# TencentYoutuResearch/NeRF-Loc

Measured on AMD Instinct MI355X. Metric: rendered rays/sec (4096 rays×128 samples, 256-wide MLP) at 1/2/4/8 MI355X, higher is better.
Workload: dtype f16mx (neural-point kernel, conv_out and feat_mlp.0: fp16 hi.hi + two MX-FP6 cross terms, 1.5 MFMA-equivalents per product; every other GEMM 3-term split-bf16 or split-fp16; fp32 accumulate; meets 1e-4)

## Files before the change

### nerf_loc_amd/csrc/tgemm.hip

```cpp
#include "common.h"
#include "mfma.h"

namespace {

__device__ __forceinline__ void tg_split8_f16(const float (&v)[8], nl_bf16x8& hi, nl_bf16x8& lo) {
  nl_f16x8 h, l;
#pragma unroll
  for (int t = 0; t < 8; ++t) { const _Float16 x = (_Float16)v[t]; h[t] = x; l[t] = (_Float16)(v[t] - (float)x); }
  hi = __builtin_bit_cast(nl_bf16x8, h);
  lo = __builtin_bit_cast(nl_bf16x8, l);
}

__device__ __forceinline__ int tg_find_seg(const NlGemmArgs& a, int k0) {
  int s = 0;
#pragma unroll
  for (int j = 1; j < NL_GEMM_MAX_SEG; ++j) s += (k0 >= a.kstart[j]) ? 1 : 0;
  return __builtin_amdgcn_readfirstlane(s);
}

#ifdef TG_TRACE
__device__ unsigned long long tg_trace[64];
#define TG_T(i)                                                                                      \
  do {                                                                                               \
    if (NRT == 8 && EPI == NL_EPI_LNSLAB && blockIdx.x == 0 && wave == 0 && a.Kpad > 512) {          \
// ... 839 lines not shown
    nl_f32x2 s = {0.f, 0.f};
#pragma unroll
    for (int r = 0; r < 16; r += 2) s = __builtin_elementwise_fma(nl_lrelu2(nl_f32x2{acc[rt][r], acc[rt][r + 1]} + bb), wp[r >> 1], s);
    float p = s[0] + s[1];
    p += __shfl_xor(p, 32, 64);
    if (hh == 0) red[wave * 256 + 32 * rt + j] = p;
  }
  __syncthreads();
  const int wpr = S >> 5, rays_wg = NW / wpr, R = M / S;
  for (int i = tid; i < rays_wg * 256; i += 64 * NW) {
    const int q = i >> 8, c = i & 255;
    float sum = 0.f;
    for (int w = 0; w < wpr; ++w) sum += red[(q * wpr + w) * 256 + c];
    const int ray = grp * rays_wg + q;
    if (w2) reinterpret_cast<float*>(hcsT)[c * HB + nbuf + q] = sum;
    else if (ray < R) hc[(size_t)ray * 256 + c] = sum;
  }
  __syncthreads();
  P = Pn;
  if (w2) {
    if (nbuf == 0) grp0 = grp;
    nbuf += rays_wg;
    const bool last = grp + (int)gridDim.x >= ngroups;
    if (nbuf + rays_wg > HB || last) {
      const int n = tid % npad, set = tid / npad;
      if (set < 2 && n < C) {
        float a[8];
#pragma unroll
        for (int i = 0; i < 8; ++i) a[i] = 0.f;
#pragma unroll 8
        for (int k = 0; k < 256; ++k) {
          const float b = w2[(size_t)k * npad + n];
          const float4 h0 = hcsT[k * (HB / 4) + set * 2], h1 = hcsT[k * (HB / 4) + set * 2 + 1];
          a[0] = fmaf(h0.x, b, a[0]); a[1] = fmaf(h0.y, b, a[1]); a[2] = fmaf(h0.z, b, a[2]); a[3] = fmaf(h0.w, b, a[3]);
          a[4] = fmaf(h1.x, b, a[4]); a[5] = fmaf(h1.y, b, a[5]); a[6] = fmaf(h1.z, b, a[6]); a[7] = fmaf(h1.w, b, a[7]);
        }
        const float b2 = w2[(size_t)256 * npad + n];
#pragma unroll
        for (int i = 0; i < 8; ++i) {
          const int slot = set * 8 + i;
          const int ray = (grp0 + (slot / rays_wg) * (int)gridDim.x) * rays_wg + slot % rays_wg;
          if (slot < nbuf && ray < R) feat[(size_t)ray * C + n] = fmaf(wsum[ray], b2, a[i]);
        }
      }
      nbuf = 0;
      __syncthreads();
    }
  }
  }
}


constexpr int TGC1_NRT = 2, TGC1_NW = 4, TGC1_D = 3, TGC1_NB = TGC1_D + 1, TGC1_NCH = 24;
template <bool X3, bool F16 = false>
__global__ __launch_bounds__(64 * TGC1_NW, 4) void tgemm_conv1_kernel(const NlGemmArgs a, const char* __restrict__ p_bst, float* __restrict__ p_c, const float* __restrict__ p_zeros,
                                                                      const float* __restrict__ p_bias) {
  constexpr int NRT = TGC1_NRT, NW = TGC1_NW, D = TGC1_D, NB = TGC1_NB, NCH = TGC1_NCH;
  constexpr int PARTS = X3 ? 2 : 1;
  constexpr int CHB = 4 * NRT * 1024;
  constexpr int SLOTB = PARTS * 2 * NRT * 1024;
  constexpr int PPW = SLOTB / 1024 / NW;
  static_assert(PPW * NW * 1024 == SLOTB, "pieces per wave");
  __shared__ uint4 lds_all[NB * SLOTB / 16 + NRT * 8 * 2 + 8];
  float* sbias = reinterpret_cast<float*>(lds_all + NB * SLOTB / 16);

  const int tid = threadIdx.x, lane = tid & 63, wave = __builtin_amdgcn_readfirstlane(tid >> 6);
  const int hh = lane >> 5, j = lane & 31;
  const int tile = blockIdx.x * NW + wave;
  const int m = tile * 32 + j;
  const bool mok = m < a.M;
  const int q = m / a.So, t = m - q * a.So;

  for (int i = tid; i < NRT * 32; i += 64 * NW) sbias[i] = (p_bias && i < a.N) ? p_bias[i] : 0.f;

  const __amdgpu_buffer_rsrc_t rw = __builtin_amdgcn_make_buffer_rsrc((void*)p_bst, 0, 0x7fffffff, 0x00020000);
  const unsigned lane16 = lane * 16;
  auto stage_piece = [&](auto Cc, auto Ic) __attribute__((always_inline)) {
    constexpr int c = decltype(Cc)::value, slot = c % NB, i = decltype(Ic)::value;
    const int pp = wave + NW * i;
    unsigned so = (unsigned)c * CHB + pp * 1024;
    asm volatile("" : "+s"(so));
    __builtin_amdgcn_raw_ptr_buffer_load_lds(rw, (__attribute__((address_space(3))) void*)(lds_all + (slot * SLOTB) / 16 + pp * 64), 16, lane16, so, 0, 0);
  };
  auto stage = [&](auto Cc) __attribute__((always_inline)) {
    nl_static_for<PPW>([&](auto Ic) __attribute__((always_inline)) { stage_piece(Cc, Ic); });
  };
  const NlGemmSeg& g0 = a.seg[0];
  const int frg = __builtin_amdgcn_readfirstlane(g0.frag);
  const int fr0 = frg == 3 ? 1 : frg;
  const int cstride0 = fr0 == 1 ? 1024 : 32;
  const float* P0[3]; int okm[3];
#pragma unroll
  for (int tp = 0; tp < 3; ++tp) {
    const int i = t + tp - 1;
    const bool ok = mok && i >= 0 && i < a.Li;
    const int row = q * a.Li + i;
    okm[tp] = ok ? 1 : 0;
    const float* f = fr0 == 1 ? g0.ptr + ((size_t)(row >> 5) * (g0.k >> 4)) * 512 + ((row & 31) + 32 * hh) * 4 : g0.ptr + (size_t)row * g0.ld + (fr0 == 2 ? 4 : 8) * hh;
    P0[tp] = ok ? f : p_zeros;
  }
  auto act_off = [](int fr, int pc) __attribute__((always_inline)) { return fr == 1 ? 256 * pc : 16 * (pc >> 1) + (fr == 2 ? 8 : 4) * (pc & 1); };
  float4 raw[D][4];
  auto load_act = [&](auto Cc) __attribute__((always_inline)) {
    constexpr int c = decltype(Cc)::value, tp = c % 3, cb = c / 3;
    const float* p = P0[tp] + okm[tp] * (cb * cstride0);
#pragma unroll
    for (int pc = 0; pc < 4; ++pc) raw[c % D][pc] = *(const float4*)(p + act_off(fr0, pc));
  };
  auto load_act_piece = [&](auto Cc, auto Pc) __attribute__((always_inline)) {
    constexpr int c = decltype(Cc)::value, tp = c % 3, cb = c / 3, pc = decltype(Pc)::value;
    const float* p = P0[tp] + okm[tp] * (cb * cstride0);
    raw[c % D][pc] = *(const float4*)(p + act_off(fr0, pc));
  };

  nl_f32x16 acc[NRT];
#pragma unroll
  for (int rt = 0; rt < NRT; ++rt)
#pragma unroll
    for (int r = 0; r < 16; ++r) acc[rt][r] = 0.f;

  nl_static_for<D>([&](auto Cc) __attribute__((always_inline)) { stage(Cc); load_act(Cc); });

#if defined(TG_TRACE) && defined(TG_TRACE_C1)
#define TGC1_T(k) do { if (blockIdx.x == 0 && wave == 0 && g >= 8 && g < 14) { const unsigned long long t_ = __builtin_readcyclecounter(); if (lane == 0) tg_trace[5 * (g - 8) + (k)] = t_; } } while (0)
#else
#define TGC1_T(k)
#endif
  nl_static_for<NCH>([&](auto Gc) __attribute__((always_inline)) {
    constexpr int g = decltype(Gc)::value;
    TGC1_T(0);
    constexpr int nlater = (g + D - 1 < NCH ? D - 1 : NCH - 1 - g);
    constexpr int later = nlater * (PPW + 4);
    nl_wait_vmcnt<later>();
    TGC1_T(1);
    __syncthreads();
    TGC1_T(2);
    nl_bf16x8 bh[2], bl[2];
    {
      const float4 (&rw4)[4] = raw[g % D];
      if (fr0 == 1) {
        bh[0] = __builtin_bit_cast(nl_bf16x8, rw4[0]); bl[0] = __builtin_bit_cast(nl_bf16x8, rw4[1]);
        bh[1] = __builtin_bit_cast(nl_bf16x8, rw4[2]); bl[1] = __builtin_bit_cast(nl_bf16x8, rw4[3]);
      } else {
#pragma unroll
        for (int ks = 0; ks < 2; ++ks) {
          const float v[8] = {rw4[2 * ks].x, rw4[2 * ks].y, rw4[2 * ks].z, rw4[2 * ks].w, rw4[2 * ks + 1].x, rw4[2 * ks + 1].y, rw4[2 * ks + 1].z, rw4[2 * ks + 1].w};
          if constexpr (F16) tg_split8_f16(v, bh[ks], bl[ks]); else nl_split8<X3>(v, bh[ks], bl[ks]);
        }
      }
    }
    auto mem_slot = [&](auto Mc) __attribute__((always_inline)) {
      constexpr int m = decltype(Mc)::value;
      if constexpr (g + D < NCH) {
        if constexpr (m < PPW) stage_piece(std::integral_constant<int, g + D>{}, Mc);
        else if constexpr (m < PPW + 4) load_act_piece(std::integral_constant<int, g + D>{}, std::integral_constant<int, m - PPW>{});
      }
    };
    TGC1_T(3);
    const nl_bf16x8* L = reinterpret_cast<const nl_bf16x8*>(lds_all + ((g % NB) * SLOTB) / 16);
    nl_static_for<2 * NRT>([&](auto Tc) __attribute__((always_inline)) {
        constexpr int tt = decltype(Tc)::value, ks = tt / NRT, rt = tt % NRT;
        const nl_bf16x8 ah = L[((0 * 2 + ks) * NRT + rt) * 64 + lane];
        if (X3) {
          const nl_bf16x8 al = L[((1 * 2 + ks) * NRT + rt) * 64 + lane];
          acc[rt] = nl_mfma<F16>(al, bh[ks], acc[rt]);
          acc[rt] = nl_mfma<F16>(ah, bl[ks], acc[rt]);
        }
        acc[rt] = nl_mfma<F16>(ah, bh[ks], acc[rt]);
        mem_slot(std::integral_constant<int, (tt < 2 ? 2 * tt : 2 + tt)>{});
        if constexpr (tt < 2) mem_slot(std::integral_constant<int, 2 * tt + 1>{});
        __builtin_amdgcn_sched_barrier(0);
      });
    __builtin_amdgcn_sched_barrier(0);
    TGC1_T(4);
  });

  __syncthreads();
  float* red = sbias + NRT * 32;
  float s1 = 0.f;
#pragma unroll
  for (int rt = 0; rt < NRT; ++rt)
#pragma unroll
    for (int gq = 0; gq < 4; ++gq) {
      const int n = 32 * rt + 8 * gq + 4 * hh;
      const float4 b4 = *(const float4*)(sbias + n);
      nl_f32x2 p0, p1;
      nl_bias_sum4(acc[rt][4 * gq + 0], acc[rt][4 * gq + 1], acc[rt][4 * gq + 2], acc[rt][4 * gq + 3], b4, p0, p1, s1);
      acc[rt][4 * gq + 0] = p0[0]; acc[rt][4 * gq + 1] = p0[1]; acc[rt][4 * gq + 2] = p1[0]; acc[rt][4 * gq + 3] = p1[1];
    }
  s1 = wave_sum(s1);
  if (lane == 0) red[wave] = s1;
  __syncthreads();
  float tot = 0.f;
#pragma unroll
  for (int w = 0; w < NW; ++w) tot += red[w];
  const float cnt = (float)a.So * (float)a.N;
  const float mean = tot / cnt;
  float s2;
  {
    nl_f32x2 sp = {0.f, 0.f};
#pragma unroll
    for (int rt = 0; rt < NRT; ++rt)
#pragma unroll
      for (int r = 0; r < 16; r += 2) nl_sumsq_dev2(sp, acc[rt][r], acc[rt][r + 1], mean);
    s2 = sp[0] + sp[1];
  }
  s2 = wave_sum(s2);
  if (lane == 0) red[NW + wave] = s2;
// ... 359 lines not shown
        if constexpr (FEAT) {
#pragma unroll
          for (int rt = 0; rt < 8; ++rt) {
#pragma unroll
            for (int gq = 0; gq < 4; ++gq) {
              const int n = 32 * rt + 8 * gq + 4 * hh;
              const float4 b4 = *(const float4*)(stab + 512 + n);
              float (&v)[16] = fa[rt % (QUERY ? 4 : 8)];
              const nl_f32x2 l0 = nl_lrelu2(nl_f32x2{acc[rt][4 * gq], acc[rt][4 * gq + 1]} + nl_f32x2{b4.x, b4.y});
              const nl_f32x2 l1 = nl_lrelu2(nl_f32x2{acc[rt][4 * gq + 2], acc[rt][4 * gq + 3]} + nl_f32x2{b4.z, b4.w});
              v[4 * gq] = l0[0]; v[4 * gq + 1] = l0[1]; v[4 * gq + 2] = l1[0]; v[4 * gq + 3] = l1[1];
            }
#pragma unroll
            for (int r = 0; r < 16; ++r) acc[rt][r] = 0.f;
            if (rt >= 2) store_fa(rt - 2, rFT, row1k);
            __builtin_amdgcn_sched_barrier(0);
          }
        }
      }
      if constexpr (kd == CK_BL && Geo::last(c)) {
        const unsigned brow = mok_c ? (unsigned)m_c * 128u + 16u * hh : DROP;
#pragma unroll
        for (int gq = 0; gq < 4; ++gq)
          __builtin_amdgcn_raw_buffer_store_b128(__builtin_bit_cast(nl_u32x4, nl_f32x4{acc[0][4 * gq], acc[0][4 * gq + 1], acc[0][4 * gq + 2], acc[0][4 * gq + 3]}), rBL,
                                                 brow + 32 * gq, 0, 0);
        zero_acc(I0{}, I2{});
      }
      if constexpr (kd == CK_Q && Geo::last(c)) {
#pragma unroll
        for (int rt = 0; rt < 4; ++rt)
#pragma unroll
          for (int r = 0; r < 16; ++r) { fa[rt % (QUERY ? 4 : 8)][r] = qacc[rt % (QUERY ? 4 : 1)][r]; qacc[rt % (QUERY ? 4 : 1)][r] = 0.f; }
      }
      CHAIN_T(2);
    });
#ifdef CHAIN_TRACE
    ++trace_it;
#endif
    prev_row = QUERY ? (mok_c ? (unsigned)m_c * 512u + 16u * hh : DROP) : row1k;
    m_c = m_n; mm_c = mm_n; mok_c = mok_n;
    tile = tile_next;
    if (tile >= ntiles) break;
  }
  if constexpr (QUERY) {
#pragma unroll
    for (int q = 0; q < 16; ++q) store_fa(q, rFA, prev_row);
  } else if constexpr (FEAT) {
#pragma unroll
    for (int q = 8; q < 32; ++q) store_fa(q, rFT, prev_row);
  }
  nl_wait_vmcnt<0>();
}

}

int nl_tgemm_nrt(int N) { return N <= 64 ? 2 : (N <= 128 ? 4 : 8); }
size_t nl_tgemm_mx_image_bytes(int Kpad) { return (size_t)((Kpad / 32 + 1) / 2) * TGMX_IMG; }
size_t nl_tgemm_stream_bytes(int Kpad, int N) { return (size_t)(Kpad / 32) * 4 * nl_tgemm_nrt(N) * 1024; }

bool nl_tgemm_supported(const NlGemmArgs& a, int precision) {
  if (precision == NL_PREC_F16X3_INTERNAL && (a.epi != NL_EPI_NONE || a.tile_map)) return false;
  if (a.act == NL_ACT_LRELU_MASK && (a.epi != NL_EPI_NONE || a.So > 0 || (!a.ep_maskin && (!a.ep_res || (a.ep_ldres & 3) || (((size_t)a.ep_res) & 15))))) return false;
  if ((a.ep_maskout || a.ep_maskin) && (a.epi != NL_EPI_NONE || a.So > 0 || a.tile_map)) return false;
  if (a.ep_tab && (a.epi != NL_EPI_NONE || a.So > 0 || a.tile_map || a.act == NL_ACT_LRELU_MASK || !a.ep_tabidx || a.ep_tabK <= 0 || (a.ep_ldtab & 3) ||
                   (((size_t)a.ep_tab) & 15)))
    return false;
  if (a.tile_map && (a.epi != NL_EPI_NONE || a.So > 0 || !a.tile_count)) return false;
  if (precision == NL_PREC_F32 || !a.Bst || a.N > 256 || (a.N & 3) || (a.ldc & 3) || (((size_t)a.C) & 15) || a.M <= 0 || !a.zeros) return false;
  if (a.epi == NL_EPI_LNROW && (a.N != 32 * nl_tgemm_nrt(a.N) || a.So > 0 || !a.ep_res || (a.ep_ldres & 3) || (((size_t)a.ep_res) & 15))) return false;
  if (a.epi == NL_EPI_LNSLAB && ((a.So != 192 && a.So != 96 && a.So != 128 && a.So != 64 && a.So != 32 && a.So != 16) || a.M % a.So || a.Li != a.So || a.ostride != 1 || a.ooff != 0 || !a.ep_gamma || !a.ep_beta)) return false;
  for (int s = 0; s < a.nseg; ++s) {
    const NlGemmSeg& g = a.seg[s];
    if (!g.vec || (g.k & 31) || g.rdiv > 1 || g.ld < g.k || g.ntap < 1) return false;
    if (g.frag && precision == NL_PREC_F16X3_INTERNAL) return false;
  }
  return true;
}

static bool nl_tgemm_mx_supported(const NlGemmArgs& a, int precision) {
  if (precision != NL_PREC_BF16X3 || !a.Bsh_mx || !a.Bmx || a.epi != NL_EPI_LNSLAB || a.So != 128 || a.Li != 128 || a.N != 256 || a.ep_pool || a.tile_map) return false;
  if (a.nseg != 2 || a.Kpad != 864 || a.seg[0].k != 256 || a.seg[0].ntap != 3 || a.seg[0].ioff != 0 || a.seg[1].k != 32 || a.seg[1].ntap != 3 || a.seg[1].ioff != 0 ||
      a.seg[1].frag != 0)
    return false;
  return nl_tgemm_supported(a, precision);
}

static bool nl_tgemm_conv1_supported(const NlGemmArgs& a, int precision) {
  if ((precision != NL_PREC_BF16X3 && precision != NL_PREC_BF16) || a.epi != NL_EPI_LNSLAB || a.So != 128 || a.Li != 128 || a.N != 64 || a.tile_map || a.ep_sig_w || !a.C) return false;
  if (a.nseg != 1 || a.Kpad != 768 || a.seg[0].k != 256 || a.seg[0].ntap != 3 || a.seg[0].ioff != 0) return false;
  return nl_tgemm_supported(a, precision);
}

int nl_tgemm_launch(const NlGemmArgs& a, int precision, hipStream_t st) {
  const bool x3 = precision == NL_PREC_BF16X3;
  const int nrt = nl_tgemm_nrt(a.N);
  if (nl_tgemm_conv1_supported(a, precision)) {
    const dim3 grid((unsigned)nl_cdiv(a.M, 32 * TGC1_NW));
    if (a.seg[0].frag == 3) {
      if (!x3 || !a.Bsh16) return NL_ERR_UNSUPPORTED;
      hipLaunchKernelGGL((tgemm_conv1_kernel<true, true>), grid, dim3(64 * TGC1_NW), 0, st, a, (const char*)a.Bsh16, a.C, a.zeros, a.bias);
    } else if (x3) hipLaunchKernelGGL(tgemm_conv1_kernel<true>, grid, dim3(64 * TGC1_NW), 0, st, a, (const char*)a.Bst, a.C, a.zeros, a.bias);
    else hipLaunchKernelGGL(tgemm_conv1_kernel<false>, grid, dim3(64 * TGC1_NW), 0, st, a, (const char*)a.Bst, a.C, a.zeros, a.bias);
    return hipPeekAtLastError() == hipSuccess ? NL_OK : NL_ERR_HIP;
  }
  if (nl_tgemm_mx_supported(a, precision)) {
    hipLaunchKernelGGL(tgemm_mx_kernel, dim3((unsigned)nl_cdiv(a.M, 32 * TGMX_NW)), dim3(64 * TGMX_NW), 0, st, a, (const char*)a.Bsh_mx, (const char*)a.Bmx, a.C, a.zeros, a.bias);
// ... 24 lines not shown
    else { if (x3) NL_TG6(2, true); else NL_TG6(2, false); }
#undef NL_TG6
    return hipPeekAtLastError() == hipSuccess ? NL_OK : NL_ERR_HIP;
  }
  if (nrt == 8) { if (x3) NL_TG(8, 4, true); else NL_TG(8, 4, false); }
  else if (nrt == 4) { if (x3) NL_TG(4, 4, true); else NL_TG(4, 4, false); }
  else { if (x3) NL_TG(2, 4, true); else NL_TG(2, 4, false); }
#undef NL_TG
  return hipPeekAtLastError() == hipSuccess ? NL_OK : NL_ERR_HIP;
}

#ifdef TG_TRACE
extern "C" __attribute__((visibility("default"))) int nl_debug_tg_trace(unsigned long long* out) {
  return hipMemcpyFromSymbol(out, HIP_SYMBOL(tg_trace), sizeof(unsigned long long) * 64) == hipSuccess ? 0 : -1;
}
#endif
#ifdef CHAIN_TRACE
extern "C" __attribute__((visibility("default"))) int nl_debug_chain_trace(unsigned long long* out) {
  return hipMemcpyFromSymbol(out, HIP_SYMBOL(chain_trace), sizeof(unsigned long long) * 2 * 4 * 96) == hipSuccess ? 0 : -1;
}
#endif

namespace {
int chain_grid(int ntiles, dim3* grid) {
  const int num_cu = nl_persistent_cus();
  if (num_cu < 0) return num_cu;
  *grid = dim3(ntiles < num_cu ? nl_xcd_grid(ntiles) : num_cu);
  return NL_OK;
}
}

int nl_launch_sample_chain(const float* O, const float* T64, const float* wscale, const float* gamma, const float* beta, float eps, const void* wbase,
                           size_t off_g2, const float* bias_g2, size_t off_fc, size_t off_f0, size_t off_ba, const float* bias_f0, float* FA, float* fth,
                           float* blA, int64_t M, int precision, hipStream_t st, bool frag_out, bool frag_f16) {
  if (M <= 0) return NL_OK;
  if ((int64_t)(M + 31) * 1024 > 0x7fffffffll) return NL_ERR_UNSUPPORTED;
  const int ntiles = (int)nl_cdiv(M, 128);
  dim3 grid;
  if (chain_grid(ntiles, &grid) != NL_OK) return NL_ERR_HIP;
  NlChainArgs a{};
  a.O = O; a.T64 = T64; a.wscale = wscale; a.gamma = gamma; a.beta = beta; a.eps = eps; a.wbase = (const char*)wbase;
  a.off_g2 = (unsigned)off_g2; a.off_fc = (unsigned)off_fc; a.off_f0 = (unsigned)off_f0; a.off_ba = (unsigned)off_ba;
  a.bias_g2 = bias_g2; a.bias_f0 = bias_f0; a.FA = FA; a.fth = fth; a.blA = blA; a.M = (int)M;
  const bool x3 = precision == NL_PREC_BF16X3;
#define NL_CHAIN(FR)                                                                                                            \
  do {                                                                                                                          \
    if (x3 && fth) hipLaunchKernelGGL((sample_chain_kernel<true, true, false, FR>), grid, dim3(256), 0, st, a, ntiles);         \
    else if (x3) hipLaunchKernelGGL((sample_chain_kernel<true, false, false, FR>), grid, dim3(256), 0, st, a, ntiles);          \
    else if (fth) hipLaunchKernelGGL((sample_chain_kernel<false, true, false, FR>), grid, dim3(256), 0, st, a, ntiles);         \
    else hipLaunchKernelGGL((sample_chain_kernel<false, false, false, FR>), grid, dim3(256), 0, st, a, ntiles);                 \
  } while (0)
  if (frag_f16) {
    if (!x3 || fth || !frag_out) return NL_ERR_UNSUPPORTED;
    hipLaunchKernelGGL((sample_chain_kernel<true, false, false, true, true>), grid, dim3(256), 0, st, a, ntiles);
  } else if (frag_out) NL_CHAIN(true); else NL_CHAIN(false);
#undef NL_CHAIN
  return hipPeekAtLastError() == hipSuccess ? NL_OK : NL_ERR_HIP;
}

int nl_launch_query_chain(const float* T64, const void* wbase, size_t off_g2, const float* bias_g2, size_t off_q, float* Q, int64_t M, int precision,
                          hipStream_t st) {
  if (M <= 0) return NL_OK;
  if ((int64_t)M * 1024 > 0x7fffffffll) return NL_ERR_UNSUPPORTED;
  const int ntiles = (int)nl_cdiv(M, 128);
  dim3 grid;
  if (chain_grid(ntiles, &grid) != NL_OK) return NL_ERR_HIP;
  NlChainArgs a{};
  a.wbase = (const char*)wbase; a.M = (int)M; a.T64 = T64; a.off_g2 = (unsigned)off_g2; a.off_q = (unsigned)off_q; a.bias_g2 = bias_g2; a.Q = Q;
  if (precision == NL_PREC_BF16X3) hipLaunchKernelGGL((sample_chain_kernel<true, false, true>), grid, dim3(256), 0, st, a, ntiles);
  else hipLaunchKernelGGL((sample_chain_kernel<false, false, true>), grid, dim3(256), 0, st, a, ntiles);
  return hipPeekAtLastError() == hipSuccess ? NL_OK : NL_ERR_HIP;
}

bool nl_feat_comp_mx_supported(int W, int S, int64_t N) {
  if (W != 256 || S < 32 || (S & 31) || N <= 0 || (N & 31) || N % S || N * 256 > 0x7fffffffll * 4) return false;
  const int wpr = S >> 5;
  return (8 % wpr) == 0 || (6 % wpr) == 0;
}
int nl_launch_feat_comp_mx(const float* fa_frag, const float* wts, int64_t N, int S, const void* bsh, const void* bmx, const float* bias, float* hc, hipStream_t st,
                           const float* w2, int npad, int C, const float* wsum, float* feat, bool frag_f16) {
  if (!nl_feat_comp_mx_supported(256, S, N) || !fa_frag || !wts || !bsh || !bmx || !bias || !hc || (((size_t)wts) & 15)) return NL_ERR_UNSUPPORTED;
  if (w2 && (npad <= 0 || npad > 192 || C <= 0 || C > npad || !wsum || !feat)) return NL_ERR_UNSUPPORTED;
  const int wpr = S >> 5, nw = (8 % wpr) == 0 ? 8 : 6;
  const int ngroups = (int)nl_cdiv(N, 32 * nw);
  dim3 grid;
  if (chain_grid(ngroups, &grid) != NL_OK) return NL_ERR_HIP;
  if (nw == 8) hipLaunchKernelGGL(feat_comp_mx_kernel<8>, grid, dim3(64 * 8), 0, st, fa_frag, wts, (int)N, S, (const char*)bsh, (const char*)bmx, bias, hc, ngroups, w2, npad, C, wsum,
                                    feat, frag_f16 ? 1 : 0);
  else hipLaunchKernelGGL(feat_comp_mx_kernel<6>, grid, dim3(64 * 6), 0, st, fa_frag, wts, (int)N, S, (const char*)bsh, (const char*)bmx, bias, hc, ngroups, w2, npad, C, wsum, feat, frag_f16 ? 1 : 0);
  return hipPeekAtLastError() == hipSuccess ? NL_OK : NL_ERR_HIP;
}
```

### nerf_loc_amd/csrc/render.hip

```cpp
#include <stddef.h>
#include <stdlib.h>
#include <string.h>
#include <vector>
#include <mutex>
#include <unordered_map>
#include "common.h"
#include "host.h"
using namespace nlhost;

namespace {

void carve_mv(Bump& b, const nl_config* c, int V, int64_t N, MvBufs& m) {
  m.vis = b.take<float>((size_t)V * N); m.dd = b.take<float>((size_t)V * N);
  m.g393 = b.take<float>((size_t)N * ldg_of(c->C)); m.t64 = b.take<float>((size_t)N * 64);
}
void carve_pt(Bump& b, const nl_config* c, int64_t N, int K, PtBufs& p, bool force_generic = false) {
  const int W = c->W;
  p.idx = b.take<int>((size_t)N * K); p.d2 = b.take<float>((size_t)N * K);
  if (!force_generic && nl_point_fused_supported(W, c->precision)) { p.X = p.H1 = p.H2 = p.KV = nullptr; }
  else {
    p.X = b.take<float>((size_t)N * K * ldx_of(c->C));
    p.H1 = b.take<float>((size_t)N * K * W); p.H2 = b.take<float>((size_t)N * K * W);
    p.KV = b.take<float>((size_t)N * K * 256);
  }
// ... 20 lines not shown

void carve_hd(Bump& b, const nl_config* c, int V, int64_t R, HdBufs& h) {
  const size_t N = (size_t)R * c->S;
  h.sigma = b.take<float>(N); h.fth = b.take<float>(N * c->W); h.hc = b.take<float>((size_t)R * c->W); h.wsum = b.take<float>((size_t)R);
  h.blA = b.take<float>(N * 32); h.rgb_s = b.take<float>(N * 3);
  h.n_alive = b.take<int>((size_t)R); h.tile_list = b.take<int>(N / 32 + 2); h.tile_count = b.take<int>(1);
}

inline bool front_path(const nl_config* c, int V) {
  return c->precision != NL_PREC_F32 && nl_mv_front_supported(c->C, V, 1);
}

void carve_render(Bump& b, const nl_config* c, int V, int64_t R, RenderBufs& rb) {
  const size_t N = (size_t)R * c->S;
  rb.xyz = b.take<float>(N * 3); rb.z = b.take<float>(N);
  rb.G = b.take<float>(N * c->W);
  rb.bl1 = front_path(c, V) ? nullptr : b.take<float>(N * V * 32);
  rb.rgbv = b.take<float>(N * V * 4);
  rb.valid_s = b.take<int>(N);
  rb.FA = b.take<float>(N * c->W); rb.geo = b.take<float>(N * c->W);
  carve_mv(b, c, V, N, rb.mv); carve_pt(b, c, N, 8, rb.pt); carve_un(b, c, R, rb.un); carve_hd(b, c, V, R, rb.hd);
}

int do_mv(const Ctx& x, const nl_frame* f, const float* qc, const float* xyz, int64_t N, float* G, float* rgb_feat,
          float* vis_ang, int* valid_s, float* bl1, float* rgbv, const MvBufs& m, bool skip_g = false, const float* qrows = nullptr, int qS = 1,
          bool front = false) {
  const NlViews vw = with_query(f, qc, qrows, qS);
  if (bl1 || front) NL_TRY(ensure_pfeat(x, f));
  if (x.c->precision == NL_PREC_F32) NL_TRY(nl_launch_mv_vis(vw, f->visf_hwc, x.p<float>(x.L.dec_w), xyz, N, m.vis, m.dd, x.st));
  else NL_TRY(nl_launch_mv_vis_mfma(vw, f->visf_hwc, x.p<char>(x.L.dec_mfma), xyz, N, m.vis, m.dd, x.c->precision == NL_PREC_BF16X3, x.st));
  if (front) {
    NL_TRY(nl_launch_mv_front(vw, f->views_dev, f->images, f->feat, xyz, N, m.vis, m.dd, x.p<char>(x.L.mvf_pack), m.t64, valid_s, rgbv, x.st));
    if (skip_g) return NL_OK;
    SegSpec s1{m.t64, 64, 64, 0, 1};
    NL_TRY(run_gemm(x, G_OUTFC2, &s1, 1, N, G, x.c->W, NL_ACT_ELU));
    return NL_OK;
  }
  NL_TRY(nl_launch_mv_stats(vw, f->views_dev, f->images, f->feat, f->C, xyz, N, m.vis, m.dd, m.g393, ldg_of(f->C), rgb_feat, vis_ang, valid_s, f->pfeat,
                            x.p<float>(x.L.blw), bl1, rgbv, x.st));
  SegSpec s0{m.g393, ldg_of(f->C), ldg_of(f->C), 0, 1};
  NL_TRY(run_gemm(x, G_OUTFC0, &s0, 1, N, m.t64, 64, NL_ACT_ELU));
  if (skip_g) return NL_OK;
  SegSpec s1{m.t64, 64, 64, 0, 1};
  NL_TRY(run_gemm(x, G_OUTFC2, &s1, 1, N, G, x.c->W, NL_ACT_ELU));
  return NL_OK;
}

int do_point(const Ctx& x, const nl_frame* f, const float* xyz, const float* dir, int dir_stride, int dir_div, const float* G, int64_t N, int K,
             float* FA, const PtBufs& p, SideJoin* knn_done = nullptr, const ChainOut* chain = nullptr) {
  const int W = x.c->W, F = f->C + 3;
  const bool fused_path = K == 8 && nl_point_fused_supported(W, x.c->precision);
  if (!knn_done) NL_TRY(nl_knn_search(&f->grid, xyz, N, K, p.idx, p.d2, x.st));
  const float* t64 = chain ? chain->t64 : nullptr;
  if (t64) {
    NL_TRY(nl_launch_query_chain(t64, x.pk, x.L.bst[G_OUTFC2], x.p<float>(x.L.bias[G_OUTFC2]), x.L.bst[G_QP], p.Q, N, x.c->precision, x.st));
  } else {
    SegSpec sg{G, W, W, 0, 1};
    NL_TRY(run_gemm(x, G_Q, &sg, 1, N, p.Q, 128, NL_ACT_NONE));
  }
  if (knn_done) NL_TRY(knn_done->join());
  if (fused_path) {
    NL_TRY(ensure_ptt(x, f));
    if (!knn_done) NL_TRY(nl_launch_wscale(p.idx, p.d2, f->sp_conf, N, K, f->M, p.wscale, x.st));
    NlPointFusedArgs a;
    a.xyz = xyz; a.dir = dir; a.dir_stride = dir_stride; a.dir_div = dir_div > 0 ? dir_div : 1;
    a.idx = p.idx; a.Q = p.Q; a.O = p.O; a.ptt = f->ptt; a.sp_xyz = f->sp_xyz; a.sp_dir = f->sp_dir;
    a.wstream = x.p<uint4>(x.L.pt_stream); a.bias = x.p<float>(x.L.pt_bias); a.rd_w = x.p<float>(x.L.rd_w);
    const bool mx = x.mx && x.c->precision == NL_PREC_BF16X3 && nl_point_fused2_supported(W, x.c->precision);
    a.wstream2 = x.p<uint4>(mx ? x.L.pt_stream2_mx : x.L.pt_stream2);
    a.N = (int)N; a.M = (int)(f->M > 0x7fffffff ? 0x7fffffff : f->M); a.inv_span = 1.f / (f->views.far_ - f->views.near_);
    hipEvent_t pe0 = nullptr, pe1 = nullptr;
    if (prof_arm(&pe0, &pe1)) NL_CHECK_HIP(hipEventRecord(pe0, x.st));
    a.logit_amax = reinterpret_cast<unsigned*>(f->views_dev + 249);
    int rc2 = NL_ERR_UNSUPPORTED;
    if (nl_point_fused2_supported(W, x.c->precision)) rc2 = nl_launch_point_fused2(a, W, x.c->precision, x.st, mx, nullptr, nullptr, reinterpret_cast<unsigned*>(f->views_dev + 249),
                                                                                   reinterpret_cast<unsigned long long*>(f->views_dev + 250));
    if (rc2 == NL_ERR_UNSUPPORTED) rc2 = nl_launch_point_fused(a, W, x.c->precision, x.st);
    NL_TRY(rc2);
    if (pe1) NL_CHECK_HIP(hipEventRecord(pe1, x.st));
  } else {
    if (!p.X) return NL_ERR_UNSUPPORTED;
    NL_TRY(nl_launch_point_encode(xyz, dir, dir_stride, dir_div, N, K, f->M, p.idx, p.d2, f->sp_xyz, f->sp_feat, F, f->sp_conf, f->sp_dir,
                                  x.p<float>(x.L.rd_w), 1.f / (f->views.far_ - f->views.near_), p.X, ldx_of(f->C), p.wscale, x.st));
    const int64_t MK = N * K;
    SegSpec sx{p.X, ldx_of(f->C), F + 90, 0, 1};
    NL_TRY(run_gemm(x, G_BASE0, &sx, 1, MK, p.H1, W, NL_ACT_LRELU));
    SegSpec s1{p.H1, W, W, 0, 1}, s2{p.H2, W, W, 0, 1};
    NL_TRY(run_gemm(x, G_BASE2, &s1, 1, MK, p.H2, W, NL_ACT_LRELU));
    NL_TRY(run_gemm(x, G_BASE4, &s2, 1, MK, p.H1, W, NL_ACT_LRELU));
    NL_TRY(run_gemm(x, G_KV, &s1, 1, MK, p.KV, 256, NL_ACT_NONE));
    NL_TRY(nl_launch_attn(p.Q, p.KV, N, K, p.O, x.st, reinterpret_cast<unsigned*>(f->views_dev + 249)));
  }
  if (chain && chain->done) *chain->done = false;
  if (t64) {
    NL_TRY(nl_launch_sample_chain(p.O, t64, p.wscale, x.p<float>(x.L.ln_g), x.p<float>(x.L.ln_b), 1e-6f, x.pk, x.L.bst[G_OUTFC2],
                                  x.p<float>(x.L.bias[G_OUTFC2]), x.L.bst[G_FC], x.L.bst[G_FEAT0P], chain->fa_f16 ? x.L.bsh[G_BLENDAP] : x.L.bst[G_BLENDAP],
                                  x.p<float>(x.L.bias[G_FEAT0P]), FA, chain->fth, chain->blA, N, x.c->precision, x.st, chain->fa_frag, chain->fa_f16));
    if (chain->done) *chain->done = true;
    return NL_OK;
  }
  SegSpec so{p.O, 128, 128, 0, 1};
  const RowEpi ep{G, W, x.p<float>(x.L.ln_g), x.p<float>(x.L.ln_b), p.wscale, 1e-6f, FA};
  bool fused = false;
  NL_TRY(run_gemm(x, G_FC, &so, 1, N, p.FCo, W, NL_ACT_NONE, 0, 0, 0, 1, 0, &ep, &fused));
  if (!fused) NL_TRY(nl_launch_ln_agg(p.FCo, G, N, W, x.p<float>(x.L.ln_g), x.p<float>(x.L.ln_b), 1e-6f, p.wscale, FA, x.st));
  return NL_OK;
}

}

namespace nlhost {

int do_unet(const Ctx& x, const float* in, int64_t R, float* geo, const UnBufs& u, float* sigma_out, bool* sigma_done,
// ... 434 lines not shown
```

Before: 584,900.

## Share conv1 tap activations across lanes via DPP instead of reloading per tap

```diff
diff --git a/nerf_loc_amd/csrc/tgemm.hip b/nerf_loc_amd/csrc/tgemm.hip
--- a/nerf_loc_amd/csrc/tgemm.hip
+++ b/nerf_loc_amd/csrc/tgemm.hip
@@ -915,6 +915,14 @@
 
 
 constexpr int TGC1_NRT = 2, TGC1_NW = 4, TGC1_D = 3, TGC1_NB = TGC1_D + 1, TGC1_NCH = 24;
+constexpr int tgc1_w(int i, int ppw) { return i + TGC1_D < TGC1_NCH ? ppw : 0; }
+constexpr int tgc1_rows(int i) { return (i % 3 != 2 && i / 3 + 1 < TGC1_NCH / 3) ? 4 : 0; }
+constexpr int tgc1_later(int g, int ppw) {
+  int n = 0;
+  if (g < TGC1_D) { n = (TGC1_D - 1 - g) * ppw; for (int i = 0; i < g; ++i) n += tgc1_w(i, ppw) + tgc1_rows(i); }
+  else { n = tgc1_rows(g - TGC1_D); for (int i = g - TGC1_D + 1; i < g; ++i) n += tgc1_w(i, ppw) + tgc1_rows(i); }
+  return n;
+}
 template <bool X3, bool F16 = false>
 __global__ __launch_bounds__(64 * TGC1_NW, 4) void tgemm_conv1_kernel(const NlGemmArgs a, const char* __restrict__ p_bst, float* __restrict__ p_c, const float* __restrict__ p_zeros,
                                                                       const float* __restrict__ p_bias) {
@@ -952,28 +960,40 @@
   const int frg = __builtin_amdgcn_readfirstlane(g0.frag);
   const int fr0 = frg == 3 ? 1 : frg;
   const int cstride0 = fr0 == 1 ? 1024 : 32;
-  const float* P0[3]; int okm[3];
-#pragma unroll
-  for (int tp = 0; tp < 3; ++tp) {
-    const int i = t + tp - 1;
-    const bool ok = mok && i >= 0 && i < a.Li;
+  auto row_ptr = [&](int i) __attribute__((always_inline)) -> const float* {
     const int row = q * a.Li + i;
-    okm[tp] = ok ? 1 : 0;
-    const float* f = fr0 == 1 ? g0.ptr + ((size_t)(row >> 5) * (g0.k >> 4)) * 512 + ((row & 31) + 32 * hh) * 4 : g0.ptr + (size_t)row * g0.ld + (fr0 == 2 ? 4 : 8) * hh;
-    P0[tp] = ok ? f : p_zeros;
-  }
+    return fr0 == 1 ? g0.ptr + ((size_t)(row >> 5) * (g0.k >> 4)) * 512 + ((row & 31) + 32 * hh) * 4 : g0.ptr + (size_t)row * g0.ld + (fr0 == 2 ? 4 : 8) * hh;
+  };
+  const int te = j == 0 ? t - 1 : t + 1;
+  const bool oke = mok && (j == 0 || j == 31) && te >= 0 && te < a.Li;
+  const float* Pcen = mok ? row_ptr(t) : p_zeros;
+  const float* Pedge = oke ? row_ptr(te) : p_zeros;
+  const int okc = mok ? 1 : 0, okE = oke ? 1 : 0;
   auto act_off = [](int fr, int pc) __attribute__((always_inline)) { return fr == 1 ? 256 * pc : 16 * (pc >> 1) + (fr == 2 ? 8 : 4) * (pc & 1); };
-  float4 raw[D][4];
-  auto load_act = [&](auto Cc) __attribute__((always_inline)) {
-    constexpr int c = decltype(Cc)::value, tp = c % 3, cb = c / 3;
-    const float* p = P0[tp] + okm[tp] * (cb * cstride0);
-#pragma unroll
-    for (int pc = 0; pc < 4; ++pc) raw[c % D][pc] = *(const float4*)(p + act_off(fr0, pc));
-  };
-  auto load_act_piece = [&](auto Cc, auto Pc) __attribute__((always_inline)) {
-    constexpr int c = decltype(Cc)::value, tp = c % 3, cb = c / 3, pc = decltype(Pc)::value;
-    const float* p = P0[tp] + okm[tp] * (cb * cstride0);
-    raw[c % D][pc] = *(const float4*)(p + act_off(fr0, pc));
+  constexpr int NCB = NCH / 3;
+  float4 cen[2][4];
+  float4 edge[4];
+  auto load_cen_piece = [&](auto CBc, auto Pc) __attribute__((always_inline)) {
+    constexpr int cb = decltype(CBc)::value, pc = decltype(Pc)::value;
+    cen[cb % 2][pc] = *(const float4*)(Pcen + okc * (cb * cstride0) + act_off(fr0, pc));
+  };
+  auto load_edge_piece = [&](auto CBc, auto Pc) __attribute__((always_inline)) {
+    constexpr int cb = decltype(CBc)::value, pc = decltype(Pc)::value;
+    edge[pc] = *(const float4*)(Pedge + okE * (cb * cstride0) + act_off(fr0, pc));
+  };
+  auto tap_words = [&](auto CBc, auto TPc, float4 (&w)[4]) __attribute__((always_inline)) {
+    constexpr int cb = decltype(CBc)::value, tp = decltype(TPc)::value;
+#pragma unroll
+    for (int pc = 0; pc < 4; ++pc) {
+      const float4 c4 = cen[cb % 2][pc], e4 = edge[pc];
+      if constexpr (tp == 1) w[pc] = c4;
+      else {
+        constexpr int CTRL = tp == 0 ? 0x138 : 0x130;
+        const bool fix = lane == (tp == 0 ? 32 : 31);
+        const float dx = nl_dpp<CTRL>(c4.x, e4.x), dy = nl_dpp<CTRL>(c4.y, e4.y), dz = nl_dpp<CTRL>(c4.z, e4.z), dw = nl_dpp<CTRL>(c4.w, e4.w);
+        w[pc] = float4{fix ? e4.x : dx, fix ? e4.y : dy, fix ? e4.z : dz, fix ? e4.w : dw};
+      }
+    }
   };
 
   nl_f32x16 acc[NRT];
@@ -981,8 +1001,11 @@
   for (int rt = 0; rt < NRT; ++rt)
 #pragma unroll
     for (int r = 0; r < 16; ++r) acc[rt][r] = 0.f;
-
-  nl_static_for<D>([&](auto Cc) __attribute__((always_inline)) { stage(Cc); load_act(Cc); });
+  nl_bf16x8 bh2[2], bl2[2];
+
+  nl_static_for<4>([&](auto Pc) __attribute__((always_inline)) { load_cen_piece(std::integral_constant<int, 0>{}, Pc); });
+  nl_static_for<4>([&](auto Pc) __attribute__((always_inline)) { load_edge_piece(std::integral_constant<int, 0>{}, Pc); });
+  nl_static_for<D>([&](auto Cc) __attribute__((always_inline)) { stage(Cc); });
 
 #if defined(TG_TRACE) && defined(TG_TRACE_C1)
 #define TGC1_T(k) do { if (blockIdx.x == 0 && wave == 0 && g >= 8 && g < 14) { const unsigned long long t_ = __builtin_readcyclecounter(); if (lane == 0) tg_trace[5 * (g - 8) + (k)] = t_; } } while (0)
@@ -992,31 +1015,35 @@
   nl_static_for<NCH>([&](auto Gc) __attribute__((always_inline)) {
     constexpr int g = decltype(Gc)::value;
     TGC1_T(0);
-    constexpr int nlater = (g + D - 1 < NCH ? D - 1 : NCH - 1 - g);
-    constexpr int later = nlater * (PPW + 4);
-    nl_wait_vmcnt<later>();
+    constexpr int cb = g / 3, tp = g % 3;
+    nl_wait_vmcnt<tgc1_later(g, PPW)>();
     TGC1_T(1);
     __syncthreads();
     TGC1_T(2);
-    nl_bf16x8 bh[2], bl[2];
-    {
-      const float4 (&rw4)[4] = raw[g % D];
-      if (fr0 == 1) {
-        bh[0] = __builtin_bit_cast(nl_bf16x8, rw4[0]); bl[0] = __builtin_bit_cast(nl_bf16x8, rw4[1]);
-        bh[1] = __builtin_bit_cast(nl_bf16x8, rw4[2]); bl[1] = __builtin_bit_cast(nl_bf16x8, rw4[3]);
+    auto operand = [&](auto TPc, nl_bf16x8 (&oh)[2], nl_bf16x8 (&ol)[2]) __attribute__((always_inline)) {
+      float4 rw4[4];
+      tap_words(std::integral_constant<int, cb>{}, TPc, rw4);
+      if (F16 || fr0 == 1) {
+        oh[0] = __builtin_bit_cast(nl_bf16x8, rw4[0]); ol[0] = __builtin_bit_cast(nl_bf16x8, rw4[1]);
+        oh[1] = __builtin_bit_cast(nl_bf16x8, rw4[2]); ol[1] = __builtin_bit_cast(nl_bf16x8, rw4[3]);
       } else {
 #pragma unroll
         for (int ks = 0; ks < 2; ++ks) {
           const float v[8] = {rw4[2 * ks].x, rw4[2 * ks].y, rw4[2 * ks].z, rw4[2 * ks].w, rw4[2 * ks + 1].x, rw4[2 * ks + 1].y, rw4[2 * ks + 1].z, rw4[2 * ks + 1].w};
-          if constexpr (F16) tg_split8_f16(v, bh[ks], bl[ks]); else nl_split8<X3>(v, bh[ks], bl[ks]);
-        }
-      }
-    }
+          if constexpr (F16) tg_split8_f16(v, oh[ks], ol[ks]); else nl_split8<X3>(v, oh[ks], ol[ks]);
+        }
+      }
+    };
+    nl_bf16x8 bh[2], bl[2];
+    if constexpr (tp == 2) { bh[0] = bh2[0]; bh[1] = bh2[1]; bl[0] = bl2[0]; bl[1] = bl2[1]; }
+    else operand(std::integral_constant<int, tp>{}, bh, bl);
+    if constexpr (tp == 1) operand(std::integral_constant<int, 2>{}, bh2, bl2);
     auto mem_slot = [&](auto Mc) __attribute__((always_inline)) {
       constexpr int m = decltype(Mc)::value;
-      if constexpr (g + D < NCH) {
-        if constexpr (m < PPW) stage_piece(std::integral_constant<int, g + D>{}, Mc);
-        else if constexpr (m < PPW + 4) load_act_piece(std::integral_constant<int, g + D>{}, std::integral_constant<int, m - PPW>{});
+      if constexpr (m < PPW) { if constexpr (g + D < NCH) stage_piece(std::integral_constant<int, g + D>{}, Mc); }
+      else if constexpr (m < PPW + 4 && cb + 1 < NCB) {
+        if constexpr (tp == 0) load_cen_piece(std::integral_constant<int, cb + 1>{}, std::integral_constant<int, m - PPW>{});
+        if constexpr (tp == 1) load_edge_piece(std::integral_constant<int, cb + 1>{}, std::integral_constant<int, m - PPW>{});
       }
     };
     TGC1_T(3);
```

Result: no change. 584,700 (-0.0%).

## Add 8-wave sample chain kernel sharing LDS weight ring across 256-row tiles

Applied to the files above, without the earlier changes.

```diff
diff --git a/nerf_loc_amd/csrc/render.hip b/nerf_loc_amd/csrc/render.hip
--- a/nerf_loc_amd/csrc/render.hip
+++ b/nerf_loc_amd/csrc/render.hip
@@ -96,13 +96,13 @@
   const bool fused_path = K == 8 && nl_point_fused_supported(W, x.c->precision);
   if (!knn_done) NL_TRY(nl_knn_search(&f->grid, xyz, N, K, p.idx, p.d2, x.st));
   const float* t64 = chain ? chain->t64 : nullptr;
+  if (knn_done) NL_TRY(knn_done->join());
   if (t64) {
     NL_TRY(nl_launch_query_chain(t64, x.pk, x.L.bst[G_OUTFC2], x.p<float>(x.L.bias[G_OUTFC2]), x.L.bst[G_QP], p.Q, N, x.c->precision, x.st));
   } else {
     SegSpec sg{G, W, W, 0, 1};
     NL_TRY(run_gemm(x, G_Q, &sg, 1, N, p.Q, 128, NL_ACT_NONE));
   }
-  if (knn_done) NL_TRY(knn_done->join());
   if (fused_path) {
     NL_TRY(ensure_ptt(x, f));
     if (!knn_done) NL_TRY(nl_launch_wscale(p.idx, p.d2, f->sp_conf, N, K, f->M, p.wscale, x.st));
diff --git a/nerf_loc_amd/csrc/tgemm.hip b/nerf_loc_amd/csrc/tgemm.hip
--- a/nerf_loc_amd/csrc/tgemm.hip
+++ b/nerf_loc_amd/csrc/tgemm.hip
@@ -1482,6 +1482,228 @@
   nl_wait_vmcnt<0>();
 }
 
+struct Chain2wGeo {
+  static constexpr int NCH = 8;
+  static constexpr int cm(int c) { return ((c % NCH) + NCH) % NCH; }
+  static constexpr int kind(int c) { return cm(c) < 2 ? CK_G2 : cm(c) < 6 ? CK_FC : CK_BL; }
+  static constexpr int idx(int c) { return cm(c) < 2 ? cm(c) : cm(c) < 6 ? cm(c) - 2 : cm(c) - 6; }
+  static constexpr int post(int c) {
+    const int k = kind(c), i = idx(c);
+    if (k == CK_G2) return 4;
+    if (k == CK_FC) return i < 2 ? 4 : i == 3 ? 1 : 0;
+    return 4 * 5 + (i == 1 ? 4 : 0);
+  }
+};
+
+__global__ __launch_bounds__(512, 2) void sample_chain2w_kernel(const NlChainArgs a, const int ntiles) {
+  using Geo = Chain2wGeo;
+  __builtin_amdgcn_s_setreg(1473, 1);
+  constexpr int NW = 8, NB = 4, NCH = Geo::NCH;
+  constexpr int SLOT16 = 2 * 2 * 8 * 64;
+  constexpr int PPW = 2 * 2 * 8 / NW;
+  [[maybe_unused]] constexpr bool QUERY = false;
+  __shared__ uint4 lds_all[NB * SLOT16 + 3 * 64];
+  nl_bf16x8 (*ring)[SLOT16] = reinterpret_cast<nl_bf16x8 (*)[SLOT16]>(lds_all);
+  float* stab = reinterpret_cast<float*>(lds_all + NB * SLOT16);
+  const int tid = threadIdx.x, lane = tid & 63, wave = __builtin_amdgcn_readfirstlane(tid >> 6);
+  const int hh = lane >> 5, j = lane & 31;
+  int tile = (int)nl_xcd_block();
+  if (tile >= ntiles) return;
+  constexpr unsigned DROP = 0x80000000u;
+  const __amdgpu_buffer_rsrc_t rFA = __builtin_amdgcn_make_buffer_rsrc((void*)a.FA, 0, ((a.M + 31) >> 5) * 32768, 0x00020000);
+  const __amdgpu_buffer_rsrc_t rBL = __builtin_amdgcn_make_buffer_rsrc((void*)a.blA, 0, a.M * 128, 0x00020000);
+  if (tid < 256) { stab[tid] = a.gamma[tid]; stab[256 + tid] = a.beta[tid]; stab[512 + tid] = a.bias_g2[tid]; }
+
+  const __amdgpu_buffer_rsrc_t rw = __builtin_amdgcn_make_buffer_rsrc((void*)a.wbase, 0, 0x7fffffff, 0x00020000);
+  const unsigned wvoff = wave * 1024 + lane * 16;
+  uint4* lw = lds_all + wave * 64;
+  auto dma_chunk = [&](auto Cc) __attribute__((always_inline)) {
+    constexpr int c = Geo::cm(decltype(Cc)::value), kd = Geo::kind(c);
+    const unsigned so = (kd == CK_FC ? a.off_fc : kd == CK_BL ? a.off_ba : a.off_g2) + (unsigned)(Geo::idx(c) * 32768);
+    nl_static_for<PPW>([&](auto Ic) __attribute__((always_inline)) {
+      constexpr int i = decltype(Ic)::value;
+      unsigned s2 = so + i * (NW * 1024);
+      asm volatile("" : "+s"(s2));
+      __builtin_amdgcn_raw_ptr_buffer_load_lds(rw, (__attribute__((address_space(3))) void*)(lw + (c % NB) * SLOT16 + i * (NW * 64)), 16, wvoff, s2, 0, 0);
+    });
+  };
+
+  nl_f32x16 acc[8], bacc;
+  nl_f32x4 oraw[8];
+  nl_f32x4 traw[8];
+  auto row_of = [&](int t, int& m, int& mm, bool& mok) __attribute__((always_inline)) {
+    m = t * (32 * NW) + 32 * wave + j;
+    mok = m < a.M;
+    mm = mok ? m : a.M - 1;
+  };
+  auto load_traw = [&](int i, int mm) __attribute__((always_inline)) {
+    traw[i] = *reinterpret_cast<const nl_f32x4*>(a.T64 + (size_t)mm * 64 + 8 * hh + 16 * (i >> 1) + 4 * (i & 1));
+  };
+  auto load_oraw = [&](int i, int mm) __attribute__((always_inline)) {
+    oraw[i % 8] = *reinterpret_cast<const nl_f32x4*>(a.O + (size_t)mm * 128 + 8 * hh + 16 * (i >> 1) + 4 * (i & 1));
+  };
+
+#pragma unroll
+  for (int rt = 0; rt < 8; ++rt)
+#pragma unroll
+    for (int r = 0; r < 16; ++r) acc[rt][r] = 0.f;
+#pragma unroll
+  for (int r = 0; r < 16; ++r) bacc[r] = 0.f;
+
+  dma_chunk(std::integral_constant<int, 0>{}); dma_chunk(std::integral_constant<int, 1>{}); dma_chunk(std::integral_constant<int, 2>{});
+  int m_c, mm_c; bool mok_c;
+  row_of(tile, m_c, mm_c, mok_c);
+#pragma unroll
+  for (int i = 0; i < 8; ++i) load_traw(i, mm_c);
+#ifdef CHAIN_TRACE
+  int trace_it = 0;
+#endif
+  float mean = 0.f, rstd = 0.f, sc = 0.f;
+  nl_wait_vmcnt<0>();
+  __syncthreads();
+
+  for (;;) {
+    const int tile_next = tile + (int)gridDim.x;
+    int m_n, mm_n; bool mok_n;
+    row_of(tile_next < ntiles ? tile_next : tile, m_n, mm_n, mok_n);
+    const unsigned fragoff = (unsigned)(tile * NW + wave) * 32768u + (unsigned)lane * 16u;
+    nl_static_for<NCH>([&](auto Cc) __attribute__((always_inline)) {
+      constexpr int c = decltype(Cc)::value, kd = Geo::kind(c), g = Geo::idx(c);
+      constexpr int younger = 2 * PPW + Geo::post(c - 3) + Geo::post(c - 2) + Geo::post(c - 1);
+      static_assert(younger < 63, "vmcnt is a 6-bit counter");
+      CHAIN_T(0);
+      nl_wait_vmcnt<younger>();
+      __builtin_amdgcn_s_barrier();
+      CHAIN_T(1);
+      dma_chunk(std::integral_constant<int, c + 3>{});
+      __builtin_amdgcn_sched_barrier(0);
+
+      if constexpr (kd != CK_BL) {
+        nl_bf16x8 bh[2], bl[2];
+#pragma unroll
+        for (int ks = 0; ks < 2; ++ks) {
+          nl_f32x4 u0, u1;
+          if constexpr (kd == CK_FC) { u0 = oraw[(4 * g + 2 * ks) % 8]; u1 = oraw[(4 * g + 2 * ks + 1) % 8]; }
+          else { u0 = traw[4 * g + 2 * ks]; u1 = traw[4 * g + 2 * ks + 1]; }
+          const float v[8] = {u0[0], u0[1], u0[2], u0[3], u1[0], u1[1], u1[2], u1[3]};
+          nl_split8<true>(v, bh[ks], bl[ks]);
+        }
+        const nl_bf16x8* L = ring[c % NB];
+        auto ldA = [&](int tt, nl_bf16x8& ah, nl_bf16x8& al) __attribute__((always_inline)) {
+          const int ks = tt >> 3, rt = tt & 7;
+          ah = L[((0 * 2 + ks) * 8 + rt) * 64 + lane];
+          al = L[((1 * 2 + ks) * 8 + rt) * 64 + lane];
+        };
+        nl_bf16x8 ah[3], al[3];
+        ldA(0, ah[0], al[0]);
+        ldA(1, ah[1], al[1]);
+#pragma unroll
+        for (int tt = 0; tt < 16; ++tt) {
+          if (tt + 2 < 16) ldA(tt + 2, ah[(tt + 2) % 3], al[(tt + 2) % 3]);
+          const int ks = tt >> 3, rt = tt & 7;
+          acc[rt] = __builtin_amdgcn_mfma_f32_32x32x16_bf16(al[tt % 3], bh[ks], acc[rt], 0, 0, 0);
+          acc[rt] = __builtin_amdgcn_mfma_f32_32x32x16_bf16(ah[tt % 3], bl[ks], acc[rt], 0, 0, 0);
+          acc[rt] = __builtin_amdgcn_mfma_f32_32x32x16_bf16(ah[tt % 3], bh[ks], acc[rt], 0, 0, 0);
+          if ((tt & 3) == 1) {
+            const int k = tt >> 2;
+            if constexpr (kd == CK_G2) load_oraw(4 * g + k, mm_c);
+            else if constexpr (g < 2) load_oraw(8 + 4 * g + k, mm_c);
+          }
+          __builtin_amdgcn_sched_barrier(0);
+        }
+        if constexpr (kd == CK_G2 && g == 1) {
+#pragma unroll
+          for (int rt = 0; rt < 8; ++rt) {
+#pragma unroll
+            for (int gq = 0; gq < 4; ++gq) {
+              const float4 b4 = *(const float4*)(stab + 512 + 32 * rt + 8 * gq + 4 * hh);
+              const nl_f32x2 e0 = nl_elu_fast2(nl_f32x2{acc[rt][4 * gq + 0], acc[rt][4 * gq + 1]} + nl_f32x2{b4.x, b4.y});
+              const nl_f32x2 e1 = nl_elu_fast2(nl_f32x2{acc[rt][4 * gq + 2], acc[rt][4 * gq + 3]} + nl_f32x2{b4.z, b4.w});
+              acc[rt][4 * gq + 0] = e0[0]; acc[rt][4 * gq + 1] = e0[1]; acc[rt][4 * gq + 2] = e1[0]; acc[rt][4 * gq + 3] = e1[1];
+            }
+            __builtin_amdgcn_sched_barrier(0);
+          }
+        }
+        if constexpr (kd == CK_FC && g == 3) {
+          nl_f32x2 sp1 = {0.f, 0.f};
+#pragma unroll
+          for (int rt = 0; rt < 8; ++rt)
+#pragma unroll
+            for (int r = 0; r < 16; r += 4) sp1 += nl_f32x2{acc[rt][r], acc[rt][r + 1]} + nl_f32x2{acc[rt][r + 2], acc[rt][r + 3]};
+          float s1 = sp1[0] + sp1[1];
+          s1 += __shfl_xor(s1, 32, 64);
+          mean = s1 / 256.f;
+          nl_f32x2 sp2 = {0.f, 0.f};
+#pragma unroll
+          for (int rt = 0; rt < 8; ++rt)
+#pragma unroll
+            for (int r = 0; r < 16; r += 2) nl_sumsq_dev2(sp2, acc[rt][r], acc[rt][r + 1], mean);
+          float s2 = sp2[0] + sp2[1];
+          s2 += __shfl_xor(s2, 32, 64);
+          rstd = 1.f / sqrtf(s2 / 256.f + a.eps);
+          sc = a.wscale[mm_c];
+        }
+      } else {
+        nl_static_for<4>([&](auto Sc) __attribute__((always_inline)) {
+          constexpr int sub = decltype(Sc)::value, kc = 4 * g + sub;
+          load_traw(kc, mm_n);
+          __builtin_amdgcn_sched_barrier(0);
+          float v[16];
+#pragma unroll
+          for (int gq = 0; gq < 4; ++gq) {
+            const int n = 32 * kc + 8 * gq + 4 * hh;
+            const float4 g4 = *(const float4*)(stab + n), be4 = *(const float4*)(stab + 256 + n);
+            const nl_f32x2 mm = {mean, mean}, rr = {rstd, rstd}, ss = {sc, sc};
+            const nl_f32x2 p0 = ((nl_f32x2{acc[kc][4 * gq + 0], acc[kc][4 * gq + 1]} - mm) * rr * nl_f32x2{g4.x, g4.y} + nl_f32x2{be4.x, be4.y}) * ss;
+            const nl_f32x2 p1 = ((nl_f32x2{acc[kc][4 * gq + 2], acc[kc][4 * gq + 3]} - mm) * rr * nl_f32x2{g4.z, g4.w} + nl_f32x2{be4.z, be4.w}) * ss;
+            v[4 * gq + 0] = p0[0]; v[4 * gq + 1] = p0[1]; v[4 * gq + 2] = p1[0]; v[4 * gq + 3] = p1[1];
+          }
+          nl_bf16x8 xh[2], xl[2];
+#pragma unroll
+          for (int sI = 0; sI < 2; ++sI) {
+            const float u[8] = {v[8 * sI], v[8 * sI + 1], v[8 * sI + 2], v[8 * sI + 3], v[8 * sI + 4], v[8 * sI + 5], v[8 * sI + 6], v[8 * sI + 7]};
+            tg_split8_f16_pk(u, xh[sI], xl[sI]);
+          }
+#pragma unroll
+          for (int r = 0; r < 16; ++r) acc[kc][r] = 0.f;
+          const nl_bf16x8* L = ring[c % NB] + sub * (2 * 2 * 2 * 64);
+          __builtin_amdgcn_sched_barrier(0);
+          nl_bf16x8 wh[2], wl[2];
+#pragma unroll
+          for (int ks = 0; ks < 2; ++ks) { wh[ks] = L[((0 * 2 + ks) * 2 + 0) * 64 + lane]; wl[ks] = L[((1 * 2 + ks) * 2 + 0) * 64 + lane]; }
+          __builtin_amdgcn_sched_barrier(0);
+#pragma unroll
+          for (int ks = 0; ks < 2; ++ks) {
+            bacc = __builtin_amdgcn_mfma_f32_32x32x16_f16(__builtin_bit_cast(nl_f16x8, wl[ks]), __builtin_bit_cast(nl_f16x8, xh[ks]), bacc, 0, 0, 0);
+            bacc = __builtin_amdgcn_mfma_f32_32x32x16_f16(__builtin_bit_cast(nl_f16x8, wh[ks]), __builtin_bit_cast(nl_f16x8, xl[ks]), bacc, 0, 0, 0);
+            bacc = __builtin_amdgcn_mfma_f32_32x32x16_f16(__builtin_bit_cast(nl_f16x8, wh[ks]), __builtin_bit_cast(nl_f16x8, xh[ks]), bacc, 0, 0, 0);
+            __builtin_amdgcn_raw_buffer_store_b128(__builtin_bit_cast(nl_u32x4, xh[ks]), rFA, fragoff + (unsigned)(((2 * kc + ks) * 2 + 0) * 1024), 0, 0);
+            __builtin_amdgcn_raw_buffer_store_b128(__builtin_bit_cast(nl_u32x4, xl[ks]), rFA, fragoff + (unsigned)(((2 * kc + ks) * 2 + 1) * 1024), 0, 0);
+            __builtin_amdgcn_sched_barrier(0);
+          }
+        });
+        if constexpr (g == 1) {
+          const unsigned brow = mok_c ? (unsigned)m_c * 128u + 16u * hh : DROP;
+#pragma unroll
+          for (int gq = 0; gq < 4; ++gq)
+            __builtin_amdgcn_raw_buffer_store_b128(__builtin_bit_cast(nl_u32x4, nl_f32x4{bacc[4 * gq], bacc[4 * gq + 1], bacc[4 * gq + 2], bacc[4 * gq + 3]}), rBL,
+                                                   brow + 32 * gq, 0, 0);
+#pragma unroll
+          for (int r = 0; r < 16; ++r) bacc[r] = 0.f;
+        }
+      }
+      CHAIN_T(2);
+    });
+#ifdef CHAIN_TRACE
+    ++trace_it;
+#endif
+    m_c = m_n; mm_c = mm_n; mok_c = mok_n;
+    tile = tile_next;
+    if (tile >= ntiles) break;
+  }
+  nl_wait_vmcnt<0>();
+}
+
 }
 
 int nl_tgemm_nrt(int N) { return N <= 64 ? 2 : (N <= 128 ? 4 : 8); }
@@ -1612,7 +1834,9 @@
   } while (0)
   if (frag_f16) {
     if (!x3 || fth || !frag_out) return NL_ERR_UNSUPPORTED;
-    hipLaunchKernelGGL((sample_chain_kernel<true, false, false, true, true>), grid, dim3(256), 0, st, a, ntiles);
+    const int ntiles2 = (int)nl_cdiv(M, 256);
+    if (chain_grid(ntiles2, &grid) != NL_OK) return NL_ERR_HIP;
+    hipLaunchKernelGGL(sample_chain2w_kernel, grid, dim3(512), 0, st, a, ntiles2);
   } else if (frag_out) NL_CHAIN(true); else NL_CHAIN(false);
 #undef NL_CHAIN
   return hipPeekAtLastError() == hipSuccess ? NL_OK : NL_ERR_HIP;
```

New measurement: 578,000 before, 582,800 after, median of 6. Within noise of the previous version (+0.8%).
